# sriramelango/optimized-diffusion-model

Measured on AMD Instinct MI355X. Metric: trajectories/sec (1000-step PC sampler, NCSN++ [1,9,9], bs=128/GPU), higher is better.
Workload: dtype f32; 1 GPU; NCSN++ nf=64 ch_mult=[1,2,2] on [128,1,9,9] per GPU, 1000-step reflected PC sampler (predictor euler_maruyama, corrector none), classifier-free guidance on (2B-sample forwards), fp32; global_batch=128, num_scales=1000, score_evals_per_traj=999, parallelism=single GPU

## Files before the change

optimized-diffusion-model_amd/csrc/rdmi.hip:

```cpp
#include <hip/hip_runtime.h>

#include <algorithm>
#include <cmath>
#include <cstdarg>
#include <cstdio>
#include <cstdlib>
#include <cstring>
#include <climits>
#include <map>
#include <memory>
#include <stdexcept>
#include <string>
#include <vector>

#include "../../include/rdmi.h"
#include "attn_kernel.h"
#include "conv_kernel.h"
#include "misc_kernels.h"
#include "unet_kernel.h"
#include "bwd_kernels.h"
#include "opt_kernels.h"
#include "ode_kernels.h"
#include "tiled_kernels.h"

// ... 1506 lines not shown
            case 3: return launch_conv_t<4, 1, 1, 2, 1, 4, true>(a, s);
        }
        return fail("bad conv cfg %d", cfg);
    }
    switch (cfg) {
        case 0: return launch_conv_t<1, 4, 1, 6, 1, 2, false>(a, s);
        case 1: return launch_conv_t<2, 2, 1, 3, 1, 3, false>(a, s);
        case 2: return launch_conv_t<1, 2, 2, 1, 1, 6, false>(a, s);
        case 3: return launch_conv_t<4, 1, 1, 2, 1, 4, false>(a, s);
    }
    return fail("bad conv cfg %d", cfg);
}

const char* cfg_name(int cfg) {
    static const char* n[] = {"conv_mfma<1,4,1,6,1>", "conv_mfma<2,2,1,3,1>", "conv_mfma<1,2,2,1,1>", "conv_mfma<4,1,1,2,1>"};
    return n[cfg];
}

int launch_attn(const AttnArgs& a, hipStream_t s) {
    static bool attr_set = false;
    auto k = attn_mfma_kernel<64>;
    if (!attr_set) { HIP_OK(hipFuncSetAttribute(reinterpret_cast<const void*>(k), hipFuncAttributeMaxDynamicSharedMemorySize, 160 * 1024)); attr_set = true; }
    hipLaunchKernelGGL(k, dim3((unsigned)a.NB), dim3(RDMI_THREADS), attn_lds_bytes<64>(a.Lpad, a.G), s, a);
    HIP_OK(hipGetLastError());
    return 0;
}

const float* P(rdmi_ctx* c, const std::string& name) { return c->params[(size_t)c->pindex.at(name)].ptr; }

int do_repack(rdmi_ctx* c, hipStream_t s) {
    for (size_t i = 0; i < c->jobs.size(); ++i) {
        const Param& p = c->params[(size_t)c->job_param[i]];
        if (!p.ptr) return fail("parameter '%s' was never bound (rdmi_set_param)", p.name.c_str());
        c->jobs[i].src = p.ptr;
        const int p2 = i < c->job_param2.size() ? c->job_param2[i] : -1;
        c->jobs[i].src2 = p2 >= 0 ? c->params[(size_t)p2].ptr : nullptr;
        if (p2 >= 0 && !c->jobs[i].src2) return fail("parameter '%s' was never bound (rdmi_set_param)", c->params[(size_t)p2].name.c_str());
    }
    for (auto& p : c->params)
        if (!p.ptr) return fail("parameter '%s' was never bound (rdmi_set_param)", p.name.c_str());
    HIP_OK(hipMemcpyAsync(c->d_jobs.get(), c->jobs.data(), c->jobs.size() * sizeof(PackJob), hipMemcpyHostToDevice, s));
    {
        ProfScope ps(c, s, "pack_kernel", 0);
        hipLaunchKernelGGL(pack_kernel, dim3(32, (unsigned)c->jobs.size()), dim3(RDMI_THREADS), 0, s, (const PackJob*)c->d_jobs.get());
    }
    HIP_OK(hipGetLastError());
    for (auto& op : c->ops) {
        if (op.kind == OP_CONV) {
            ConvArgs& a = op.conv;
            a.bias = P(c, op.p_bias);
            a.bias_sc = op.p_bias_sc.empty() ? nullptr : P(c, op.p_bias_sc);
            a.gamma = op.p_gamma.empty() ? nullptr : P(c, op.p_gamma);
            a.beta = op.p_beta.empty() ? nullptr : P(c, op.p_beta);
        } else {
            op.attn.gamma = P(c, op.p_gamma); op.attn.beta = P(c, op.p_beta); op.attn.b3 = P(c, op.p_b3);
        }
    }
    if (c->tiled) tiled_bind_params(c);
    for (auto& q : c->progs) {
        if (!q.ok) continue;
        for (auto& f : q.fpatch) {
            FOp& o = q.fprog[(size_t)f.op];
            const float* p = f.param.empty() ? c->d_w.get() + f.arena_off : P(c, f.param);
            switch (f.field) {
                case FusedBuilder::F_GAMMA: o.gamma = p; break;
                case FusedBuilder::F_BETA: o.beta = p; break;
                case FusedBuilder::F_BIAS: case FusedBuilder::F_BIAS_ARENA: o.bias = p; break;
                case FusedBuilder::F_BIAS2: o.bias2 = p; break;
                case FusedBuilder::F_W: o.main_ph.w = p; break;
                case FusedBuilder::F_SC0W: o.sc[0].w = p; break;
                case FusedBuilder::F_SC1W: o.sc[1].w = p; break;
            }
        }
        HIP_OK(hipMemcpyAsync(q.d_fprog.get(), q.fprog.data(), q.fprog.size() * sizeof(FOp), hipMemcpyHostToDevice, s));
    }
    if (c->fused_ready()) HIP_OK(hipStreamSynchronize(s));
    c->packed_valid = true;
    return 0;
}

struct FwdIn {
    const float* x; int x_mod;
    const float* sig; int sig_mod;
    float t_scalar;
    int t_is_time; float smin, ratio;
    const float* labels; int label_rows;
    float* out; int NB;
    const float* tt_row = nullptr;
    const float* dense_rows = nullptr;
    float drop_p = 0.f; const unsigned long long* seed_dev = nullptr;
};

}
#include "tiled_plan.h"
namespace {

int run_forward(rdmi_ctx* c, const FwdIn& f, hipStream_t s) {
    const rdmi_arch& a = c->arch;
    if (f.NB < 1 || f.NB > c->max_batch) return fail("batch %d outside [1, %d] (rdmi_create max_batch)", f.NB, c->max_batch);
    if (a.scale_by_sigma && !c->tiled) return fail("scale_by_sigma=True is only built for the tiled plan (the shipped GTO-Halo config sets it False, RD/configs/model/ncsnpp.yaml)");
    if (a.conditional && !f.labels) return fail("class_labels is required: the model is conditional (label_emb) -- reference raises here too (RD/models/ncsnpp.py:262)");
    const int T = c->temb, Np_t = (T + 63) & ~63, Np_d = (c->dense_total + 63) & ~63;
    if (!f.tt_row && !f.dense_rows) {
    LinArgs l{};
    l.M = f.NB; l.fourW = P(c, "time_embed.W"); l.nfour = a.nf;
    l.X = f.sig; l.x_mod = f.sig_mod > 0 ? f.sig_mod : f.NB; l.t_is_time = f.t_is_time; l.smin = f.smin; l.ratio = f.ratio;
    l.use_scalar = f.sig ? 0 : 1; l.t_scalar = f.t_scalar;
    l.pre = 2; l.K = pad16(2 * a.nf); l.W = c->d_w.get() + c->w_t0; l.Npad = Np_t; l.N = T; l.bias = P(c, "time_mlp.0.bias");
    l.Y = c->d_h1.get(); l.ldy = T;
    {
        ProfScope ps(c, s, "linear_mfma(time_mlp.0)", 2.0 * f.NB * T * 2 * a.nf);
        hipLaunchKernelGGL(linear_mfma_kernel<1>, dim3((unsigned)ceil_div(f.NB, 16), (unsigned)(Np_t / 64)), dim3(RDMI_THREADS), 0, s, l);
    }
    LinArgs l2{};
    l2.M = f.NB; l2.X = c->d_h1.get(); l2.ldx = T; l2.pre = 1; l2.K = T; l2.W = c->d_w.get() + c->w_t2; l2.Npad = Np_t; l2.N = T;
    l2.bias = P(c, "time_mlp.2.bias"); l2.Y = c->d_temb.get(); l2.ldy = T;
    if (a.conditional) { l2.labels = f.labels; l2.Wl = P(c, "label_emb.weight"); l2.bl = P(c, "label_emb.bias"); l2.ncls = a.num_classes; l2.label_rows = f.label_rows; }
    {
        ProfScope ps(c, s, "linear_mfma(time_mlp.2)", 2.0 * f.NB * T * T);
        hipLaunchKernelGGL(linear_mfma_kernel<1>, dim3((unsigned)ceil_div(f.NB, 16), (unsigned)(Np_t / 64)), dim3(RDMI_THREADS), 0, s, l2);
    }
    }
    if (!f.dense_rows) {
    LinArgs l3{};
    l3.M = f.NB; l3.X = c->d_temb.get(); l3.ldx = T; l3.pre = 1; l3.K = T;
    if (f.tt_row) {
        l3.X = f.tt_row; l3.ldx = 0; l3.pre = 3;
        if (a.conditional) { l3.labels = f.labels; l3.Wl = P(c, "label_emb.weight"); l3.ncls = a.num_classes; l3.label_rows = f.label_rows; }
    } l3.W = c->d_w.get() + c->w_dense; l3.Npad = Np_d; l3.N = c->dense_total;
    l3.bias = c->d_w.get() + c->b_dense; l3.Y = c->d_dense.get(); l3.ldy = c->dense_total;
    {
        ProfScope ps(c, s, "linear_mfma(Dense_0 x all)", 2.0 * f.NB * T * c->dense_total);
        hipLaunchKernelGGL((linear_mfma_kernel<1, 16>), dim3((unsigned)ceil_div(f.NB, 16), (unsigned)(Np_d / 64)), dim3(RDMI_THREADS), 0, s, l3);
    }
    }
    HIP_OK(hipGetLastError());
    if (a.compute_dtype == 1 && !c->tiled && !c->in_train_forward)
        return fail("compute_dtype=bf16 on this shape is built for the TRAINING step only (model.train_dtype = 'bf16'); sampling and evaluation of the "
                    "GTO-Halo model run the exact-fp32 plans");
    if (c->tiled) return run_tiled(c, f, s);
    const rdmi_ctx::FusedProg* fq = (c->use_fused && !c->debug_taps) ? c->pick(f.NB) : nullptr;
    if (c->in_train_forward) {
        static const int fused_upto = [] { const char* e = std::getenv("RDMI_TRAIN_FUSED_UPTO"); return e ? atoi(e) : 2 * std::max(resident_workgroups(), 1); }();
        fq = (c->train_prog >= 0 && c->progs[(size_t)c->train_prog].ok && f.NB <= fused_upto) ? &c->progs[(size_t)c->train_prog] : nullptr;
    }
    if (fq) {
        static bool attr_set = false;
        if (!attr_set) {
            HIP_OK(hipFuncSetAttribute(reinterpret_cast<const void*>(unet_wg_kernel<false>), hipFuncAttributeMaxDynamicSharedMemorySize, 160 * 1024));
            HIP_OK(hipFuncSetAttribute(reinterpret_cast<const void*>(unet_wg_kernel<true>), hipFuncAttributeMaxDynamicSharedMemorySize, 160 * 1024));
            HIP_OK(hipFuncSetAttribute(reinterpret_cast<const void*>((unet_wg_kernel<false, true>)), hipFuncAttributeMaxDynamicSharedMemorySize, 160 * 1024));
            HIP_OK(hipFuncSetAttribute(reinterpret_cast<const void*>((unet_wg_kernel<false, true, true>)), hipFuncAttributeMaxDynamicSharedMemorySize, 160 * 1024));
            HIP_OK(hipFuncSetAttribute(reinterpret_cast<const void*>((unet_wg_kernel<true, true, true>)), hipFuncAttributeMaxDynamicSharedMemorySize, 160 * 1024));
            HIP_OK(hipFuncSetAttribute(reinterpret_cast<const void*>((unet_wg_kernel<false, false, false, true>)), hipFuncAttributeMaxDynamicSharedMemorySize, 160 * 1024));
            attr_set = true;
        }
        UnetArgs ua = fq->fargs;
        ua.x_in = f.x; ua.x_mod = f.x_mod; ua.out = f.out; ua.NB = f.NB;
        unsigned nwg = (unsigned)ceil_div(f.NB, fq->S);
        if (fq->coop) {
            nwg = (unsigned)(ceil_div(ceil_div(f.NB, 4), ua.coop_stride) * 4 * ua.coop_stride);
            ua.epoch_base = c->coop_epoch;
            c->coop_epoch += (unsigned)fq->n_xchg;
            if (c->coop_epoch > 0xfff00000u) c->coop_epoch = 0;
        }
        if (f.dense_rows) ua.dense = f.dense_rows;
        double fl = 0;
        for (auto& op : c->ops) fl += op.flops_per_sample;
        ProfScope ps(c, s, "unet_wg_kernel", fl * f.NB);
        c->last_prog = (int)(fq - c->progs.data());
        if (fq->train) {
            ua.drop_p = c->train_drop_p; ua.seed_dev = c->train_seed_dev;
            hipLaunchKernelGGL((unet_wg_kernel<false, false, false, true>), dim3(nwg), dim3(UW_THREADS), fq->fused_lds, s, ua);
            HIP_OK(hipGetLastError());
            return 0;
        }
        if ((ua.stamps || ua.dbg) && fq->S == 1) hipLaunchKernelGGL(unet_wg_kernel<true>, dim3(nwg), dim3(UW_THREADS), fq->fused_lds, s, ua);
        else if ((ua.stamps || ua.dbg) && fq->coop) hipLaunchKernelGGL((unet_wg_kernel<true, true, true>), dim3(nwg), dim3(UW_THREADS), fq->fused_lds, s, ua);
        else if (fq->coop) hipLaunchKernelGGL((unet_wg_kernel<false, true, true>), dim3(nwg), dim3(UW_THREADS), fq->fused_lds, s, ua);
        else if (fq->S > 1) hipLaunchKernelGGL((unet_wg_kernel<false, true>), dim3(nwg), dim3(UW_THREADS), fq->fused_lds, s, ua);
        else hipLaunchKernelGGL(unet_wg_kernel<false>, dim3(nwg), dim3(UW_THREADS), fq->fused_lds, s, ua);
        HIP_OK(hipGetLastError());
        return 0;
    }
    for (auto& op : c->ops) {
        if (op.kind == OP_CONV) {
            ConvArgs ca = op.conv;
            ca.NB = f.NB;
            if (op.a_is_input) { ca.srcA = f.x; ca.srcA_mod = f.x_mod; }
            if (op.out_is_output) ca.out = f.out;
            if (op.use_dense && f.dense_rows) ca.dense = f.dense_rows;
            ProfScope ps(c, s, cfg_name(op.cfg), op.flops_per_sample * f.NB);
            if (int e = launch_conv(op.cfg, ca, s)) return e;
        } else {
            AttnArgs aa = op.attn;
            aa.NB = f.NB;
            ProfScope ps(c, s, "attn_mfma<64>", op.flops_per_sample * f.NB);
            if (int e = launch_attn(aa, s)) return e;
        }
    }
    return 0;
}

}

#include "train_plan.h"
#include "tiled_train.h"

TrainPlan::~TrainPlan() {
    if (side) (void)hipStreamSynchronize(side);
    if (fwd_exec) (void)hipGraphExecDestroy(fwd_exec);
    for (auto& e : bwd_exec) if (e) (void)hipGraphExecDestroy(e);
    for (int p = 0; p < 2; ++p) {
        if (ev_ready[p]) (void)hipEventDestroy(ev_ready[p]);
        if (ev_done[p]) (void)hipEventDestroy(ev_done[p]);
    }
    if (side) (void)hipStreamDestroy(side);
    if (cap) (void)hipStreamDestroy(cap);
}

rdmi_ctx::~rdmi_ctx() {
    train.reset();
    for (auto& ev : ev_pool) { (void)hipEventDestroy(ev.first); (void)hipEventDestroy(ev.second); }
}

extern "C" {

const char* rdmi_last_error(void) { return g_err.c_str(); }
int rdmi_debug_op_cycles(rdmi_ctx* c, long long* host, int cap, const char** desc, int desc_cap) {
    if (!c || !c->d_stamps || !c->fused_ready()) return 0;
    const rdmi_ctx::FusedProg& q0 = c->progs[(size_t)std::min<int>(std::max(c->last_prog, 0), (int)c->progs.size() - 1)];
    const int n = (int)q0.fprog.size();
    std::vector<long long> st((size_t)n + 1);
    if (n > 1000) return 0;
    if (hipMemcpy(st.data(), c->d_stamps.get(), st.size() * sizeof(long long), hipMemcpyDeviceToHost) != hipSuccess) return 0;
    for (int i = 0; i < n && i < cap; ++i) host[i] = st[(size_t)i + 1] - st[(size_t)i];
    {
        std::vector<long long> fs((size_t)n * 8);
        if (hipMemcpy(fs.data(), c->d_stamps.get() + 1024, fs.size() * sizeof(long long), hipMemcpyDeviceToHost) == hipSuccess)
            for (int i = 0; i < n && 256 + i * 8 + 7 < cap; ++i)
                for (int k = 0; k < 8; ++k) host[256 + i * 8 + k] = fs[(size_t)i * 8 + k] - st[(size_t)i];
    }
    for (int i = 0; i < n && i < desc_cap; ++i) desc[i] = q0.fdesc[(size_t)i].c_str();
    return n;
}

int rdmi_debug_program(rdmi_ctx* c, int prog, int* S, int* coop, int* train, const char** desc, int desc_cap) {
    if (!c || prog < 0 || prog >= (int)c->progs.size() || !c->progs[(size_t)prog].ok) return -1;
    const rdmi_ctx::FusedProg& q = c->progs[(size_t)prog];
    if (S) *S = q.S;
    if (coop) *coop = q.coop ? 1 : 0;
    if (train) *train = q.train ? 1 : 0;
    const int n = (int)q.fdesc.size();
    for (int i = 0; desc && i < n && i < desc_cap; ++i) desc[i] = q.fdesc[(size_t)i].c_str();
    return n;
}

int rdmi_debug_packed(rdmi_ctx* c, const char* key, float* dst, size_t numel, void* stream) {
    if (!c || !key || !dst) return fail("null argument");
    auto it = c->wmap.find(key);
    if (it == c->wmap.end()) return fail("no packed tensor '%s'", key);
    if (it->second + numel > c->w_floats) return fail("packed tensor '%s': %zu floats exceed the arena", key, numel);
    HIP_OK(hipMemcpyAsync(dst, c->d_w.get() + it->second, numel * sizeof(float), hipMemcpyDeviceToDevice, (hipStream_t)stream));
    return 0;
}

const char* rdmi_path_info(rdmi_ctx* c) {
    static thread_local std::string s;
    if (!c) return "";
    if (c->tiled) {
        s = std::string("tiled (") + (c->arch.compute_dtype == 1 ? "bf16 MFMA operands, fp32 accumulate" : "fp32") + "): " + std::to_string(c->tiled->launches.size()) + " launches over HBM-resident NHWC tensors (" + std::to_string(c->tiled->ws_per_sample * 4 / 1024) + " KiB of activations per sample)";
        long n_resize = 0;
        for (auto& l : c->tiled->launches) n_resize += std::holds_alternative<TResizeL>(l.op);
        s += "; resize launches (h onto an odd skip grid): " + std::to_string(n_resize);
    } else if (c->fused_ready() && c->use_fused && !c->debug_taps) {
        s = "fused: workgroup-resident U-Net, " + std::to_string(c->progs[0].fprog.size()) + " ops, " + std::to_string(c->progs[0].fused_lds) + " B LDS";
        for (size_t i = 1; i < c->progs.size(); ++i)
            if (c->progs[i].coop)
                s += c->progs[i].ok ? "; co-operative groups of 4 workgroups up to batch " + std::to_string(c->progs[i].max_nb) + " (" + std::to_string(c->progs[i].fprog.size()) + " ops, " + std::to_string(c->progs[i].n_xchg) + " exchanges, id stride " + std::to_string(c->coop_stride) + (c->use_coop ? ")" : ", disabled)")
                                    : "; co-operative program unavailable (" + c->progs[i].why + ")";
            else
            s += c->progs[i].ok ? "; S=" + std::to_string(c->progs[i].S) + " samples/workgroup from batch " + std::to_string(c->s_min_wg * c->progs[i].S) + " (" + std::to_string(c->progs[i].fprog.size()) + " ops)"
                                : "; S=" + std::to_string(c->progs[i].S) + " unavailable (" + c->progs[i].why + ")";
    } else {
        s = "layers: " + std::to_string(c->ops.size()) + " launches" + (c->fused_ready() ? "" : " (fused unavailable: " + (c->progs.empty() ? std::string("not built") : c->progs[0].why) + ")");
    }
    for (auto& q : c->progs) if (q.train && !q.ok) s += "; fused training forward unavailable (" + q.why + ")";
    if (c->train_prog >= 0 && c->progs[(size_t)c->train_prog].ok)
        s += "; training forward: fused program (" + std::to_string(c->progs[(size_t)c->train_prog].fprog.size()) + " ops, layer outputs stashed for the backward)";
    if (c->train) s += "; input-gradient backward calls: " + std::to_string(c->train->input_dgrad_calls);
    return s.c_str();
}

int rdmi_philox_normal(float* z, size_t n, unsigned long long seed, unsigned long long elem_offset, unsigned draw, void* stream) {
    if (n == 0) return 0;
    if (!z) return fail("null argument");
    hipLaunchKernelGGL(philox_normal_kernel, dim3((unsigned)((n + 4 * RDMI_THREADS - 1) / (4 * RDMI_THREADS))), dim3(RDMI_THREADS), 0, (hipStream_t)stream, z, (long)n,
                       (uint64_t)seed, (uint64_t)elem_offset, (const int*)nullptr, (int)draw);
    HIP_OK(hipGetLastError());
    return 0;
}

int rdmi_coop_status(rdmi_ctx* c, int* gave_up) {
    if (!c || !gave_up) return fail("null argument");
    *gave_up = 0;
    for (auto& q : c->progs)
        if (q.coop && q.d_coop_err) { int v = 0; HIP_OK(hipMemcpy(&v, q.d_coop_err.get(), sizeof v, hipMemcpyDeviceToHost)); *gave_up |= v; }
    if (*gave_up) c->use_coop = false;
    return 0;
}
const char* rdmi_version(void) {
#ifdef RDMI_EMU
    return "rdmi 0.1 (CPU execution-model emulator build: tests only)";
#else
    return "rdmi 0.1 (gfx950)";
#endif
}

int rdmi_create(const rdmi_arch* arch, int max_batch, int H, int W, rdmi_ctx** out) {
    if (!arch || !out) return fail("null argument");
    if (arch->n_levels < 1 || arch->n_levels > RDMI_MAX_LEVELS) return fail("n_levels=%d out of range", arch->n_levels);
    if (arch->nf % 16 != 0) return fail("nf=%d must be a multiple of 16", arch->nf);
    if (max_batch < 1 || H < 2 || W < 2) return fail("bad shape max_batch=%d H=%d W=%d", max_batch, H, W);
    rdmi_ctx* c = new rdmi_ctx();
    c->arch = *arch;
    c->max_batch = max_batch; c->H = H; c->W = W;
    c->temb = arch->nf * 4;
    if (const char* e = std::getenv("RDMI_DEBUG_TAPS")) c->debug_taps = atoi(e) != 0;
    if (const char* e = std::getenv("RDMI_PATH")) c->use_fused = std::string(e) != "layers";
    int e = 0;
    try { e = build_plan(c); } catch (const std::exception& ex) { e = fail("plan construction failed: %s", ex.what()); }
// ... 534 lines not shown
```

optimized-diffusion-model_amd/csrc/unet_kernel.h:

```cpp
#pragma once
#include <cstddef>

#include "common.h"

#define UW_THREADS 512
#define UW_WAVES 8
#ifndef UW_PF_M4
#define UW_PF_M4 4
#endif
#ifndef UW_PF_N1
#define UW_PF_N1 4
#endif
#ifndef UW_PF_KS1
#define UW_PF_KS1 4
#endif
#ifndef UW_PRIO
#define UW_PRIO 0
#endif
#ifndef UW_LIGHT_BARRIER
#define UW_LIGHT_BARRIER 0
#endif

__device__ __forceinline__ void lds_barrier() {
#if defined(__HIP_DEVICE_COMPILE__) && UW_LIGHT_BARRIER
// ... 918 lines not shown
            fconv_epi<MS, TR>(w, u, n0, mt0, WM, nt, nmt, lane, add, dadd0, daddm, acc, ps1, ps2);
            k_mt0 = mt0; k_nt = nt; k_nmt = nmt;
            if (DIAG && fine) fine[5] = clock64();
        }
    }
    if (fused_gn) {
        use_from_here(gmul); use_from_here(gadd);
        lds_barrier();
        if (DIAG && fine) fine[6] = clock64();
        if (k_nmt > 0) fconv_gn_apply<MS, TR>(w, u, n0, k_mt0, WM, k_nt, k_nmt, lane, gmul, gadd, acc, ps1, ps2);
        if (DIAG && fine) fine[7] = clock64();
    }
}

template <bool DIAG>
__device__ __forceinline__ void fop_conv_coop(const OpW& w, const UnetArgs& u, int n_grp, int m, int wave, int lane, long long* fine) {
    const int lrow = lane & 15, kq = lane >> 4;
    const int ct = wave & 1, kg = wave >> 1;
    const int nt = 2 * m + ct, col = nt * 16 + lrow;
    const int o_Cout = OPI(w, Cout), o_dense = OPI(w, dense_off), hw_shift = OPI(w, hw_shift);
    const float* o_bias = OPP(w, const float, bias); const float* o_bias2 = OPP(w, const float, bias2);
    const bool fused_gn = OPI(w, gn_off) >= 0;
    const bool finisher = kg == 0;
    float add1 = ldg1(o_bias + col), add2 = ldg1((o_bias2 ? o_bias2 : o_bias) + col);
    float gmul = ldg1((fused_gn ? OPP(w, const float, gamma) : o_bias) + col), gadd = ldg1((fused_gn ? OPP(w, const float, beta) : o_bias) + col);
    float dv = ldg1(u.dense + (size_t)max(o_dense, 0) + (o_dense >= 0 ? (size_t)min(n_grp + ((kq * 4) >> hw_shift), u.NB - 1) * u.dense_stride + col : 0));
    f32x4 acc[4];
    {
        const int spt = OPI(w, main_ph.nch) >> 2;
        if (spt == 2) fconv_main_ks<DIAG, 2>(w, u, nt, lane, fine, acc, kg);
        else if (spt == 4 && (OPI(w, main_ph.nch) & 3) == 0) fconv_main_ks<DIAG, 4>(w, u, nt, lane, fine, acc, kg);
        else fconv_main<DIAG, 1, UW_PF_KS1, false, false, true>(w, u, 0, 1, nt, lane, fine, acc, kg);
    }
    float* const dstp = lds_f(OPI(w, dst_off));
    const int drs = OPI(w, dst_rs);
    if (!finisher) {
        float* p = dstp + (size_t)(kq * 4) * drs + (((m + kg) & 3) * 32 + ct * 16 + lrow);
#pragma unroll
        for (int r = 0; r < 4; ++r) p[r * drs] = acc[0][r];
    }
    use_from_here(add1); use_from_here(add2); use_from_here(dv); use_from_here(gmul); use_from_here(gadd);
    lds_barrier();
    if (finisher) {
        f32x4 part[3];
#pragma unroll
        for (int k = 1; k < 4; ++k) {
            const float* p = dstp + (size_t)(kq * 4) * drs + (((m + k) & 3) * 32 + ct * 16 + lrow);
            for (int r = 0; r < 4; ++r) part[k - 1][r] = p[r * drs];
        }
        f32x4 v = (acc[0] + part[0]) + (part[1] + part[2]);
        if (DIAG && (u.dbg & 256)) return;
        const int o_resid = OPI(w, resid_off), o_resid_rs = OPI(w, resid_rs);
        const float o_scale = OPF(w, scale), add_all = (o_bias2 ? add1 + add2 : add1) + (o_dense >= 0 ? dv : 0.f);
        const int row0 = kq * 4;
        if (o_resid >= 0) {
            const float* rp = lds_f(o_resid) + (size_t)row0 * o_resid_rs + col;
            float rv[4];
#pragma unroll
            for (int r = 0; r < 4; ++r) rv[r] = rp[r * o_resid_rs];
#pragma unroll
            for (int r = 0; r < 4; ++r) v[r] = (v[r] + add_all + rv[r]) * o_scale;
        } else {
#pragma unroll
            for (int r = 0; r < 4; ++r) v[r] = (v[r] + add_all + 0.f) * o_scale;
        }
        if (!fused_gn || OPI(w, gn_raw) != 0) {
            float* p = dstp + (size_t)row0 * drs + col;
#pragma unroll
            for (int r = 0; r < 4; ++r) p[r * drs] = v[r];
        }
        if (fused_gn) {
            const float s1 = quad_sum((v[0] + v[1]) + (v[2] + v[3])), s2 = quad_sum((v[0] * v[0] + v[1] * v[1]) + (v[2] * v[2] + v[3] * v[3]));
            const float mean = s1 * OPF(w, inv_cnt);
            const float rstd = (1.0f / sqrtf(fmaxf(s2 * OPF(w, inv_cnt) - mean * mean, 0.f) + OPF(w, eps))) * gmul;
            const int act = OPI(w, gn_act), grs = OPI(w, gn_rs);
            float* p = lds_f(OPI(w, gn_off)) + (size_t)row0 * grs + col;
#pragma unroll
            for (int r = 0; r < 4; ++r) { const float y = (v[r] - mean) * rstd + gadd; p[r * grs] = act ? silu_f(y) : y; }
        }
    }
}

__device__ __forceinline__ void fop_xchg(const OpW& w, const UnetArgs& u, int g, int m, int tid, int* failw) {
    const int mode = OPI(w, a_hw), rows = OPI(w, rows), Cs = OPI(w, C), xi = OPI(w, xidx);
    const int d_off = OPI(w, dst_off), d_rs = OPI(w, dst_rs), s_off = OPI(w, src_off), s_rs = OPI(w, src_rs);
    const int a_off = OPI(w, a_off), a_rs = OPI(w, a_rs);
    const unsigned epoch = u.epoch_base + (unsigned)xi + 1u;
    const int csh = 31 - __builtin_clz((unsigned)Cs);
    const int half = (rows << csh) >> 1;
    const int np = s_off >= 0 ? 2 * half : half;
    const unsigned slotb = (unsigned)u.xslot * 8u;
    const unsigned gbase = (unsigned)((g * 2 + (xi & 1)) * 4) * slotb;
    const XBuf xb = xbuf_make(u.xbuf, 0x7fffffffu);
    auto at = [&](int p, int j) -> int {
        const int sel = p >= half ? 1 : 0, i = (p - sel * half) << 1, row = i >> csh, c = i & (Cs - 1);
        if (mode == 0) return ((sel ? s_off : d_off) >> 2) + row * (sel ? s_rs : d_rs) + j * Cs + c;
        return (d_off >> 2) + (j * rows + row) * d_rs + c;
    };
    typedef float f32x2 __attribute__((vector_size(8)));
    constexpr int KMAX = 1;
    const bool withhold = u.coop_break != 0 && g == 0 && m == 3 && xi == 0;
#pragma unroll
    for (int k = 0; k < KMAX; ++k) {
        const int p = tid + k * UW_THREADS;
        if (p < np && !withhold) {
            f32x2 v;
            if (mode == 0) v = *reinterpret_cast<const f32x2*>(lds_f(0) + at(p, m));
            else {
                const int i = p << 1, row = i >> csh, c = i & (Cs - 1);
                v = *reinterpret_cast<const f32x2*>(lds_f(a_off) + row * a_rs + c);
                *reinterpret_cast<f32x2*>(lds_f(0) + at(p, m)) = v;
            }
            const float v0 = v[0], v1 = v[1];
            xbuf_store16(xb, gbase + (unsigned)m * slotb + (unsigned)p * 16u, __builtin_bit_cast(unsigned, v0), __builtin_bit_cast(unsigned, v1), epoch);
        }
    }
    const int nk = (np + UW_THREADS - 1) / UW_THREADS;
    u32x4 y[3 * KMAX];
    unsigned long long spins = 0;
    bool broken = __hip_atomic_load(u.coop_err, __ATOMIC_RELAXED, __HIP_MEMORY_SCOPE_AGENT) != 0;
    if (broken) *failw = 1;
    for (; !broken;) {
#pragma unroll
        for (int k = 0; k < KMAX; ++k)
            if (k < nk) {
                const unsigned po = (unsigned)min(tid + k * UW_THREADS, np - 1) * 16u;
#pragma unroll
                for (int jj = 0; jj < 3; ++jj) y[k * 3 + jj] = xbuf_load16(xb, gbase + (unsigned)((m + 1 + jj) & 3) * slotb + po);
            }
        bool ok = true;
#pragma unroll
        for (int k = 0; k < KMAX; ++k)
            if (k < nk) {
#pragma unroll
                for (int jj = 0; jj < 3; ++jj) { const unsigned t1 = y[k * 3 + jj][1], t3 = y[k * 3 + jj][3]; ok &= t1 == epoch && t3 == epoch; }
            }
        if (ok) break;
        if (++spins > RDMI_SPIN_LIMIT) { *failw = 1; __hip_atomic_store(u.coop_err, 1, __ATOMIC_RELAXED, __HIP_MEMORY_SCOPE_AGENT); break; }
        spin_relax();
    }
#pragma unroll
    for (int k = 0; k < KMAX; ++k) {
        const int p = tid + k * UW_THREADS;
        if (!broken && k < nk && p < np) {
#pragma unroll
            for (int jj = 0; jj < 3; ++jj) {
                const unsigned a = y[k * 3 + jj][0], b = y[k * 3 + jj][2];
                *reinterpret_cast<f32x2*>(lds_f(0) + at(p, (m + 1 + jj) & 3)) = f32x2{__builtin_bit_cast(float, a), __builtin_bit_cast(float, b)};
            }
        }
    }
}

__device__ __forceinline__ void fop_attn(const OpW& w, int wave, int lane) {
    struct { int L, Lpad, q_off, k_off, vt_off, p_off, qk_rs, k_rs, ps, C, dst_off, dst_rs; float att_scale; } o;
    o.L = OPI(w, L); o.Lpad = OPI(w, Lpad); o.q_off = OPI(w, q_off); o.k_off = OPI(w, k_off); o.vt_off = OPI(w, vt_off); o.p_off = OPI(w, p_off);
    o.qk_rs = OPI(w, qk_rs); o.k_rs = OPI(w, k_rs); o.ps = OPI(w, ps); o.C = OPI(w, C); o.dst_off = OPI(w, dst_off); o.dst_rs = OPI(w, dst_rs); o.att_scale = OPF(w, att_scale);
    const int lrow = lane & 15, kq = lane >> 4;
    const int L = o.L, mtiles = o.Lpad >> 4;
    const float* Q = lds_f(o.q_off);
    const float* K = lds_f(o.k_off);
    const float* Vt = lds_f(o.vt_off);
    float* P = lds_f(o.p_off);
    const int rs = o.qk_rs, krs = o.k_rs, ps = o.ps;
    const int nchq = o.C >> 4;
    for (int mt = wave; mt < mtiles; mt += UW_WAVES) {
        f32x4 s[6];
#pragma unroll
        for (int t = 0; t < 6; ++t) s[t] = f32x4{0.f, 0.f, 0.f, 0.f};
        const int qrow = min(mt * 16 + lrow, L - 1);
        for (int ch = 0; ch < nchq; ++ch) {
            const f32x4 af = *reinterpret_cast<const f32x4*>(Q + (size_t)qrow * rs + ch * 16 + kq * 4);
#pragma unroll
            for (int t = 0; t < 6; ++t) {
                if (t < mtiles) {
                    const int krow = min(t * 16 + lrow, L - 1);
                    const f32x4 bf = *reinterpret_cast<const f32x4*>(K + (size_t)krow * krs + ch * 16 + kq * 4);
#pragma unroll
                    for (int j = 0; j < 4; ++j) s[t] = mfma16(af[j], bf[j], s[t]);
                }
            }
        }
#pragma unroll
        for (int r = 0; r < 4; ++r) {
            float mx = -3.0e38f;
#pragma unroll
            for (int t = 0; t < 6; ++t)
                if (t < mtiles && t * 16 + lrow < L) { s[t][r] *= o.att_scale; mx = fmaxf(mx, s[t][r]); }
            mx = row16_max(mx);
            float sum = 0.f;
#pragma unroll
            for (int t = 0; t < 6; ++t)
                if (t < mtiles) {
                    const float e = (t * 16 + lrow < L) ? __expf(s[t][r] - mx) : 0.f;
                    s[t][r] = e;
                    sum += e;
                }
            sum = row16_sum(sum);
            const float inv = 1.0f / sum;
            const int row = mt * 16 + kq * 4 + r;
            if (row < L) {
#pragma unroll
                for (int t = 0; t < 6; ++t)
                    if (t < mtiles) P[(size_t)row * ps + t * 16 + lrow] = s[t][r] * inv;
            }
        }
    }
    lds_barrier();
    {
        const int wn = wave & 3, wm = wave >> 2;
        const int col = wn * 16 + lrow;
        f32x4 acc[3];
#pragma unroll
        for (int i = 0; i < 3; ++i) acc[i] = f32x4{0.f, 0.f, 0.f, 0.f};
        for (int ch = 0; ch < mtiles; ++ch) {
            const f32x4 bf = *reinterpret_cast<const f32x4*>(Vt + (size_t)col * ps + ch * 16 + kq * 4);
#pragma unroll
            for (int i = 0; i < 3; ++i) {
                const int mt = wm + 2 * i;
                if (mt < mtiles) {
                    const int prow = min(mt * 16 + lrow, L - 1);
                    const f32x4 af = *reinterpret_cast<const f32x4*>(P + (size_t)prow * ps + ch * 16 + kq * 4);
#pragma unroll
                    for (int j = 0; j < 4; ++j) acc[i] = mfma16(af[j], bf[j], acc[i]);
                }
            }
        }
        float* O = lds_f(o.dst_off);
        const float* b3 = OPP(w, const float, bias);
        const int o_resid = OPI(w, resid_off), o_resid_rs = OPI(w, resid_rs);
        const float o_scale = OPF(w, scale), badd = b3 ? ldg1(b3 + col) : 0.f;
#pragma unroll
        for (int i = 0; i < 3; ++i) {
            const int mt = wm + 2 * i;
            if (mt < mtiles)
                for (int r = 0; r < 4; ++r) {
                    const int row = mt * 16 + kq * 4 + r;
                    if (row < L) {
                        float v = acc[i][r];
                        if (b3) v = (v + badd + lds_f(o_resid)[(size_t)row * o_resid_rs + col]) * o_scale;
                        O[(size_t)row * o.dst_rs + col] = v;
                    }
                }
        }
    }
}

template <bool DIAG, bool MS = false, bool COOP = false, bool TRAIN = false>
__global__ __launch_bounds__(UW_THREADS) void unet_wg_kernel(UnetArgs u) {
    const int tid = threadIdx.x, lane = tid & 63;
    const int wave = __builtin_amdgcn_readfirstlane(tid >> 6);
    int n = MS ? blockIdx.x * u.S : blockIdx.x, n_multi = n, n_spill = n, spill_cap = u.NB;
    int cg = 0, cm = 0;
    if (COOP) {
        const int st = u.coop_stride, bid = blockIdx.x, blk = bid / (4 * st), r = bid - blk * 4 * st;
        cm = r / st; cg = blk * st + (r - cm * st);
        if (cg * 4 >= u.NB) return;
        n = min(cg * 4 + cm, u.NB - 1);
        n_multi = cg * 4;
        n_spill = bid * 4; spill_cap = 0x7fffffff;
    }
    {
        const int nw = u.tab_bytes >> 2;
        const int* src = reinterpret_cast<const int*>(u.tabs);
        int* dst = reinterpret_cast<int*>(rdmi_lds + u.tab_base);
        for (int i = tid; i < nw; i += UW_THREADS) dst[i] = src[i];
        float* z = lds_f(u.zero_off);
        for (int i = tid; i < (u.zero_bytes >> 2); i += UW_THREADS) z[i] = 0.f;
    }
#if defined(__HIP_DEVICE_COMPILE__) && UW_PRIO == 1
    if (wave >= 4) __builtin_amdgcn_s_setprio(1);
#elif defined(__HIP_DEVICE_COMPILE__) && UW_PRIO == 2
    if (wave < 4) __builtin_amdgcn_s_setprio(1);
#endif
    float* stat = lds_f(u.zero_off + u.zero_bytes);
    int* const failw = reinterpret_cast<int*>(stat) + 270;
    if (COOP && tid == 0) *failw = 0;
    if (DIAG && u.stamps && n == 0 && tid == 0) u.stamps[0] = clock64();
    OpW cur = opw_load(u.prog, lane);
    OpW nxt = opw_load(u.prog + (u.nops > 1 ? 1 : 0), lane);
    f32x4 pgm = {1.f, 1.f, 1.f, 1.f}, pbt = {0.f, 0.f, 0.f, 0.f};
    gn_prefetch(cur, tid, pgm, pbt);
    for (int pc = 0; pc < u.nops; ++pc) {
        const OpW nn = opw_load(u.prog + (pc + 2 < u.nops ? pc + 2 : u.nops - 1), lane);
        long long* fine = (DIAG && u.stamps && n == 0 && tid == ((u.dbg >> 16) & 7) * 64) ? u.stamps + 1024 + pc * 8 : nullptr;
        const int kind = OPI(cur, kind);
        if (DIAG && fine) fine[2] = clock64();
        f32x4 ngm = pgm, nbt = pbt;
        if (pc + 1 < u.nops) gn_prefetch(nxt, tid, ngm, nbt);
        if (DIAG && fine) fine[3] = clock64();
        const int skip = (DIAG && u.dbg) ? ((kind == FOP_GN ? 4 : kind == FOP_CONV ? 8 : kind == FOP_ATTN ? 16 : 32) & u.dbg) : 0;
        const bool multi = MS && OPI(cur, samp) < 0;
        switch (skip ? -1 : kind) {
            case FOP_GATHER: fop_gather<MS>(cur, u, multi ? n_spill : n, multi ? spill_cap : u.NB, COOP ? cm : 0, tid); break;
            case FOP_STORE: fop_store<MS>(cur, u, multi ? n_spill : n, multi ? spill_cap : u.NB, tid); break;
            case FOP_GN: fop_gn<MS>(cur, stat, tid, pgm, pbt, DIAG ? u.dbg : 0); break;
            case FOP_CONV:
                if (COOP && OPI(cur, coop)) fop_conv_coop<DIAG>(cur, u, n_multi, cm, wave, lane, fine);
                else fop_conv<DIAG, MS && !COOP, TRAIN>(cur, u, multi ? n_multi : n, wave, lane, fine);
                break;
            case FOP_ATTN: fop_attn(cur, wave, lane); break;
            case FOP_LOADTAB: {
                const int* src = OPP(cur, const int, a_g);
                int* dst = reinterpret_cast<int*>(rdmi_lds + OPI(cur, dst_off));
                const int nw = OPI(cur, rows) >> 2;
                for (int i = tid; i < nw; i += UW_THREADS) dst[i] = src[i];
                break;
            }
            case FOP_XCHG: if (COOP) fop_xchg(cur, u, cg, cm, tid, failw); break;
            default: break;
        }
        if (kind == FOP_STORE || (kind == FOP_CONV && OPI(cur, dst_kind) == 2)) __syncthreads();
        else lds_barrier();
        if (DIAG && u.stamps && n == 0 && tid == 0) u.stamps[pc + 1] = clock64();
        cur = nxt; nxt = nn; pgm = ngm; pbt = nbt;
    }
    if (COOP && *failw) {
        const int E = (int)u.out_elems;
        for (int i = tid; i < E; i += UW_THREADS) u.out[(size_t)n * E + i] = __builtin_nanf("");
    }
}
```

Before: 185.2 trajectories/s.

## Rewrite fused attention op with software-pipelined MFMA loads and split score tiles

Replaces the in-kernel attention op with a version that double-buffers LDS operand loads around the MFMA accumulations and splits the QK^T score work into half-tiles, so more waves have work when there are more than three row tiles. The softmax pass now prefetches the next row's scores, and residual values are loaded before the PV matmul. The old attention is kept as a reference path that can be selected through a debug flag, and a diagnostic launch variant is added. This aims to hide LDS latency and balance work across the waves, at the cost of more registers per wave.

```diff
diff --git a/optimized-diffusion-model_amd/csrc/rdmi.hip b/optimized-diffusion-model_amd/csrc/rdmi.hip
--- a/optimized-diffusion-model_amd/csrc/rdmi.hip
+++ b/optimized-diffusion-model_amd/csrc/rdmi.hip
@@ -1682,6 +1682,7 @@
             HIP_OK(hipFuncSetAttribute(reinterpret_cast<const void*>((unet_wg_kernel<false, true>)), hipFuncAttributeMaxDynamicSharedMemorySize, 160 * 1024));
             HIP_OK(hipFuncSetAttribute(reinterpret_cast<const void*>((unet_wg_kernel<false, true, true>)), hipFuncAttributeMaxDynamicSharedMemorySize, 160 * 1024));
             HIP_OK(hipFuncSetAttribute(reinterpret_cast<const void*>((unet_wg_kernel<true, true, true>)), hipFuncAttributeMaxDynamicSharedMemorySize, 160 * 1024));
+            HIP_OK(hipFuncSetAttribute(reinterpret_cast<const void*>((unet_wg_kernel<true, true>)), hipFuncAttributeMaxDynamicSharedMemorySize, 160 * 1024));
             HIP_OK(hipFuncSetAttribute(reinterpret_cast<const void*>((unet_wg_kernel<false, false, false, true>)), hipFuncAttributeMaxDynamicSharedMemorySize, 160 * 1024));
             attr_set = true;
         }
@@ -1707,6 +1708,7 @@
         }
         if ((ua.stamps || ua.dbg) && fq->S == 1) hipLaunchKernelGGL(unet_wg_kernel<true>, dim3(nwg), dim3(UW_THREADS), fq->fused_lds, s, ua);
         else if ((ua.stamps || ua.dbg) && fq->coop) hipLaunchKernelGGL((unet_wg_kernel<true, true, true>), dim3(nwg), dim3(UW_THREADS), fq->fused_lds, s, ua);
+        else if (ua.dbg && fq->S > 1) hipLaunchKernelGGL((unet_wg_kernel<true, true>), dim3(nwg), dim3(UW_THREADS), fq->fused_lds, s, ua);
         else if (fq->coop) hipLaunchKernelGGL((unet_wg_kernel<false, true, true>), dim3(nwg), dim3(UW_THREADS), fq->fused_lds, s, ua);
         else if (fq->S > 1) hipLaunchKernelGGL((unet_wg_kernel<false, true>), dim3(nwg), dim3(UW_THREADS), fq->fused_lds, s, ua);
         else hipLaunchKernelGGL(unet_wg_kernel<false>, dim3(nwg), dim3(UW_THREADS), fq->fused_lds, s, ua);
diff --git a/optimized-diffusion-model_amd/csrc/unet_kernel.h b/optimized-diffusion-model_amd/csrc/unet_kernel.h
--- a/optimized-diffusion-model_amd/csrc/unet_kernel.h
+++ b/optimized-diffusion-model_amd/csrc/unet_kernel.h
@@ -1094,7 +1094,7 @@
     }
 }
 
-__device__ __forceinline__ void fop_attn(const OpW& w, int wave, int lane) {
+__device__ __forceinline__ void fop_attn_ref(const OpW& w, int wave, int lane) {
     struct { int L, Lpad, q_off, k_off, vt_off, p_off, qk_rs, k_rs, ps, C, dst_off, dst_rs; float att_scale; } o;
     o.L = OPI(w, L); o.Lpad = OPI(w, Lpad); o.q_off = OPI(w, q_off); o.k_off = OPI(w, k_off); o.vt_off = OPI(w, vt_off); o.p_off = OPI(w, p_off);
     o.qk_rs = OPI(w, qk_rs); o.k_rs = OPI(w, k_rs); o.ps = OPI(w, ps); o.C = OPI(w, C); o.dst_off = OPI(w, dst_off); o.dst_rs = OPI(w, dst_rs); o.att_scale = OPF(w, att_scale);
@@ -1186,6 +1186,143 @@
                 }
         }
     }
+}
+
+template <bool SH_IS_A>
+__device__ __forceinline__ void fattn_chunk(const f32x4& s, const f32x4 (&v)[3], f32x4& sn, f32x4 (&vn)[3], const float* sh, const float* const (&va)[3], int nx,
+                                            f32x4 (&acc)[3]) {
+#pragma unroll
+    for (int j = 0; j < 4; ++j) {
+        if (j == 0) { sn = *reinterpret_cast<const f32x4*>(sh + nx); vn[0] = *reinterpret_cast<const f32x4*>(va[0] + nx); }
+        else if (j < 3) vn[j] = *reinterpret_cast<const f32x4*>(va[j] + nx);
+        RDMI_SCHED_FENCE();
+#pragma unroll
+        for (int i = 0; i < 3; ++i) acc[i] = SH_IS_A ? mfma16(s[j], v[i][j], acc[i]) : mfma16(v[i][j], s[j], acc[i]);
+        RDMI_SCHED_FENCE();
+    }
+}
+template <bool SH_IS_A>
+__device__ __forceinline__ void fattn_mm(const float* sh, const float* const (&va)[3], int nch, f32x4 (&acc)[3]) {
+    f32x4 s0 = *reinterpret_cast<const f32x4*>(sh), v0[3], s1, v1[3];
+#pragma unroll
+    for (int i = 0; i < 3; ++i) { v0[i] = *reinterpret_cast<const f32x4*>(va[i]); acc[i] = f32x4{0.f, 0.f, 0.f, 0.f}; }
+    for (int ch = 0; ch < nch; ch += 2) {
+        fattn_chunk<SH_IS_A>(s0, v0, s1, v1, sh, va, min(ch + 1, nch - 1) * 16, acc);
+        if (ch + 1 < nch) fattn_chunk<SH_IS_A>(s1, v1, s0, v0, sh, va, min(ch + 2, nch - 1) * 16, acc);
+    }
+}
+
+template <bool DIAG>
+__device__ __forceinline__ void fop_attn(const OpW& w, int wave, int lane, long long* fine) {
+    if (DIAG && fine) fine[0] = clock64();
+    const int lrow = lane & 15, kq = lane >> 4;
+    const int L = OPI(w, L), mtiles = OPI(w, Lpad) >> 4, ps = OPI(w, ps);
+    float* P = lds_f(OPI(w, p_off));
+    {
+        const int rs = OPI(w, qk_rs), krs = OPI(w, k_rs), nchq = OPI(w, C) >> 4;
+        const float* Q = lds_f(OPI(w, q_off)) + kq * 4;
+        const float* K = lds_f(OPI(w, k_off)) + kq * 4;
+        const float att_scale = OPF(w, att_scale);
+        const int ush = mtiles > 3 ? 1 : 0;
+        for (int un = wave; un < (mtiles << ush); un += UW_WAVES) {
+            const int mt = un >> ush, t0 = (un & ush) * 3;
+            const float* kp[3];
+#pragma unroll
+            for (int t = 0; t < 3; ++t) kp[t] = K + mad_u24(min((t0 + t) * 16 + lrow, L - 1), krs, 0);
+            f32x4 s[3];
+            fattn_mm<true>(Q + mad_u24(min(mt * 16 + lrow, L - 1), rs, 0), kp, nchq, s);
+            const int row0 = mt * 16 + kq * 4;
+            float* pr = P + mad_u24(row0, ps, t0 * 16 + lrow);
+#pragma unroll
+            for (int r = 0; r < 4; ++r)
+                if (row0 + r < L) {
+#pragma unroll
+                    for (int t = 0; t < 3; ++t)
+                        if (t0 + t < mtiles) pr[r * ps + t * 16] = s[t][r] * att_scale;
+                }
+        }
+    }
+    lds_barrier();
+    if (DIAG && fine) fine[1] = clock64();
+    {
+        auto rd = [&](int row, float (&v)[6]) -> float* {
+            float* p = P + mad_u24(min(row, L - 1), ps, lrow);
+#pragma unroll
+            for (int t = 0; t < 6; ++t) v[t] = p[min(t, mtiles - 1) * 16];
+            return p;
+        };
+        float vn[6];
+        float* pn = rd(wave * 4 + kq, vn);
+        for (int row = wave * 4 + kq, it = 0; it < ((L + 31) >> 5); ++it, row += 32) {
+            float s[6];
+#pragma unroll
+            for (int t = 0; t < 6; ++t) s[t] = vn[t];
+            float* const prow = pn;
+            pn = rd(row + 32, vn);
+            float mx = -3.0e38f;
+#pragma unroll
+            for (int t = 0; t < 6; ++t)
+                if (t < mtiles && t * 16 + lrow < L) mx = fmaxf(mx, s[t]);
+            mx = row16_max(mx);
+            float sum = 0.f;
+#pragma unroll
+            for (int t = 0; t < 6; ++t)
+                if (t < mtiles) {
+                    const float e = (t * 16 + lrow < L) ? __expf(s[t] - mx) : 0.f;
+                    s[t] = e;
+                    sum += e;
+                }
+            sum = row16_sum(sum);
+            const float inv = 1.0f / sum;
+            if (row < L) {
+#pragma unroll
+                for (int t = 0; t < 6; ++t)
+                    if (t < mtiles) prow[t * 16] = s[t] * inv;
+            }
+        }
+    }
+    lds_barrier();
+    if (DIAG && fine) fine[4] = clock64();
+    {
+        const int wn = wave & 3, wm = wave >> 2;
+        const int col = wn * 16 + lrow;
+        const float* b3 = OPP(w, const float, bias);
+        const int dst_rs = OPI(w, dst_rs);
+        float* O = lds_f(OPI(w, dst_off)) + col;
+        float badd = 0.f, res[3][4];
+        if (b3) {
+            badd = ldg1(b3 + col);
+            const float* X = lds_f(OPI(w, resid_off)) + col;
+            const int xrs = OPI(w, resid_rs);
+#pragma unroll
+            for (int i = 0; i < 3; ++i)
+#pragma unroll
+                for (int r = 0; r < 4; ++r) res[i][r] = X[mad_u24(min((wm + 2 * i) * 16 + kq * 4 + r, L - 1), xrs, 0)];
+        }
+        const float* pp[3];
+#pragma unroll
+        for (int i = 0; i < 3; ++i) pp[i] = P + mad_u24(min((wm + 2 * i) * 16 + lrow, L - 1), ps, kq * 4);
+        f32x4 acc[3];
+        fattn_mm<false>(lds_f(OPI(w, vt_off)) + mad_u24(col, ps, kq * 4), pp, mtiles, acc);
+        if (DIAG && fine) fine[5] = clock64();
+        const float o_scale = OPF(w, scale);
+        float* const o0 = O + mad_u24(wm * 16 + kq * 4, dst_rs, 0);
+#pragma unroll
+        for (int i = 0; i < 3; ++i) {
+            const int mt = wm + 2 * i;
+            if (mt < mtiles) {
+#pragma unroll
+                for (int r = 0; r < 4; ++r) {
+                    if (mt * 16 + kq * 4 + r < L) {
+                        float v = acc[i][r];
+                        if (b3) v = (v + badd + res[i][r]) * o_scale;
+                        o0[(32 * i + r) * dst_rs] = v;
+                    }
+                }
+            }
+        }
+    }
+    if (DIAG && fine) fine[6] = clock64();
 }
 
 template <bool DIAG, bool MS = false, bool COOP = false, bool TRAIN = false>
@@ -1241,7 +1378,10 @@
                 if (COOP && OPI(cur, coop)) fop_conv_coop<DIAG>(cur, u, n_multi, cm, wave, lane, fine);
                 else fop_conv<DIAG, MS && !COOP, TRAIN>(cur, u, multi ? n_multi : n, wave, lane, fine);
                 break;
-            case FOP_ATTN: fop_attn(cur, wave, lane); break;
+            case FOP_ATTN:
+                if (DIAG && (u.dbg & 4096)) fop_attn_ref(cur, wave, lane);
+                else fop_attn<DIAG>(cur, wave, lane, fine);
+                break;
             case FOP_LOADTAB: {
                 const int* src = OPP(cur, const int, a_g);
                 int* dst = reinterpret_cast<int*>(rdmi_lds + OPI(cur, dst_off));
```

After: 186.1 trajectories/s, median of 6. Within noise of the previous version (+0.4%).
